# githubhjs/h264-jm-commentary

Hardware: AMD Instinct MI355X
Metric: ME+transform megapixels/sec @1080p FullSearch SR=32; bit-exact vs the in-repo JM restatement (oracle); device-resident (inputs in HBM, no H2D/D2H in the timed region) (higher is better)
Workload: dtype u8

## Files before the change

### h264-jm-commentary_amd/csrc/jmh_analyse.hip

```cpp
#include "jmh_common.h"
#include "jmh_launch.h"
#include "jmh_intra8.h"
#include "jmh_intra.h"
#include "jmh_i4.h"
#include "jmh_spiral.h"
#ifdef JMH_FLOW_TU
#include "jmh_final.h"
#endif

#define MVB_OFF 544
#define MVB_LEN 1104
#define MV_ABS_MAX (4 * 2 * SRMAX + 3)
#define MVB_ARG_MAX (4 * 2 * SRMAX + MV_ABS_MAX + 3)
static_assert(MVB_ARG_MAX == 518 && MVB_ARG_MAX <= MVB_OFF && MVB_OFF + MVB_ARG_MAX < MVB_LEN,
              "s.mvc holds every MV difference the full-pel and sub-pel searches can form at SRMAX");
#define PLS (WIN_DIM_MAX * WST + 32)
#define MAXNS 7

struct MeS {
    uint8_t org[256];
    Border bd;
    IntraNb<uint8_t> nb;
    int16_t all_mv[8][16][2];
    int motion_cost[8][4];
    unsigned red[NTA / 64][MAXNS];
    int pmv[MAXNS][2];
    uint16_t mvc[MVB_LEN];
    uint8_t planes[4 * PLS];
    union {
        int16_t h1[WIN_DIM_MAX * WST];
        uint2 sad8[NPK * NTA];
    } hs;
    gptr<unsigned long long> pst;
    int pn;
    alignas(8) IntraS<uint8_t> in;
};
union AnalyseS {
    MeS me;
    IntraS<uint8_t> in[4];
};

__device__ __forceinline__ void sstamp(MeS &s, int wave) {
    if (wave == 2 && __lane_id() == 0 && s.pst && s.pn < 44) s.pst[s.pn++] = wall_clock64();
}

struct NbMe {
    const MeS &s;
    int bt, b8, best8x8;
    __device__ bool operator()(int xN, int yN, int &ref, int &mx, int &my) const {
        if (yN > 15 || (xN > 15 && yN >= 0)) return false;
        if (xN < 0 || yN < 0) {
            int c = border_cell(xN, yN);
// ... 60 lines not shown
#pragma unroll
        for (int k = 0; k < NPK; k++) {
            const unsigned cost = psum<BT, BX, BY>(sp[k]) + cxv + cy[4 * k];
            const uint32_t o = ordk_of(ps, k);
            const bool in = max(rx, abs(ps.dy0 + k - sr)) <= range || o == 0;
            b = min(b, in ? (cost << 13) | o : 0xFFFFFFFFu);
        }
    }
    return b;
}

__device__ __forceinline__ int search_range(const DevParams &d, int bt) { return d.restrict_sr == 0 ? d.sr / min(2, bt) : d.sr; }

struct SDesc {
    int bt, bx4, by4, mc;
    int fbt, fbx4, fby4, fslot;
};

__device__ __forceinline__ uint32_t lds_u32_at(const uint8_t *p) { return lds_u32_any(p); }
typedef short s16x2 __attribute__((ext_vector_type(2)));
__device__ __forceinline__ s16x2 as_s2(uint32_t v) { return __builtin_bit_cast(s16x2, v); }
__device__ __forceinline__ uint32_t as_u32(s16x2 v) { return __builtin_bit_cast(uint32_t, v); }
__device__ __forceinline__ s16x2 abs2(s16x2 v) { return __builtin_elementwise_max(v, (s16x2)(0) - v); }
__device__ __forceinline__ s16x2 lo16(uint32_t w) { return as_s2(__builtin_amdgcn_perm(0u, w, 0x0c010c00u)); }
__device__ __forceinline__ s16x2 hi16(uint32_t w) { return as_s2(__builtin_amdgcn_perm(0u, w, 0x0c030c02u)); }
__device__ __forceinline__ s16x2 tap6_2(s16x2 a, s16x2 b, s16x2 c, s16x2 d, s16x2 e, s16x2 f) {
    return (a + f) + (s16x2)(20) * (c + d) - (s16x2)(5) * (b + e);
}
__device__ __forceinline__ s16x2 clip5(s16x2 v) {
    return __builtin_elementwise_min(__builtin_elementwise_max((v + (s16x2)(16)) >> (s16x2)(5), (s16x2)(0)), (s16x2)(255));
}
__device__ __forceinline__ uint32_t pack4(s16x2 lo, s16x2 hi) { return __builtin_amdgcn_perm(as_u32(hi), as_u32(lo), 0x06040200u); }

template <bool HALF>
__device__ __forceinline__ int subblock_satd(const MeS &s, int wbase, int obase, int ox, int oy, int had) {
    const int off = qoff((oy & 3) * 4 + (ox & 3));
    const int xa = (off >> 12) & 15, ya = (off >> 8) & 15, xb = (off >> 4) & 15, yb = off & 15;
    const int oA = ((xa & 1) + 2 * (ya & 1)) * PLS + (ya >> 1) * WST + (xa >> 1);
    const int oB = ((xb & 1) + 2 * (yb & 1)) * PLS + (yb >> 1) * WST + (xb >> 1);
    const uint8_t *r0 = s.planes + wbase + (oy >> 2) * WST + (ox >> 2);
    uint32_t O[4], P[4];
#pragma unroll
    for (int yy = 0; yy < 4; yy++) {
        const uint32_t A = lds_u32_at(r0 + yy * WST + oA);
        if constexpr (HALF) P[yy] = A;
        else {
            const uint32_t B = lds_u32_at(r0 + yy * WST + oB);
            P[yy] = (A | B) - (((A ^ B) >> 1) & 0x7F7F7F7Fu);
        }
        O[yy] = *reinterpret_cast<const uint32_t *>(s.org + obase + 16 * yy);
    }
    if (!had) {
        uint32_t sad = 0;
#pragma unroll
        for (int yy = 0; yy < 4; yy++) sad = __builtin_amdgcn_sad_u8(O[yy], P[yy], sad);
// ... 398 lines not shown
    }
    int minc = BIGCOST, c_mode = 0;
#pragma unroll
    for (int m = 0; m < 4; m++) {
        int c = 0;
#pragma unroll
        for (int q = 0; q < 8; q++) c += __builtin_amdgcn_readlane(sat, 8 * m + q);
        if (chroma_mode_ok(m, avL, avT, avTL) && c < minc) { minc = c; c_mode = m; }
    }
    if (lane == 0) scr->c_mode = c_mode;
}

template <class SC>
__device__ __forceinline__ void intra_slot(const DevParams &d, IntraS<uint8_t> &s, SC *scr, int16_t (*i4lev)[16], int k, int w, int mbx, int mby);

__device__ __forceinline__ void me_prologue(const DevParams &d, MeS &s, int mbx, int mby) {
    const int tid = threadIdx.x;
    if (tid < 256) s.in.org[tid] = s.org[tid] = d.orgY[(16 * mby + (tid >> 4)) * d.W + 16 * mbx + (tid & 15)];
    else if (tid >= 472 && tid < 478) s.in.part[(tid - 472) / 3][(tid - 472) % 3] = 0;
    else if (tid >= 480 && tid < 512) s.motion_cost[(tid - 480) >> 2][tid & 3] = 0;
    for (int i = tid; i < MVB_LEN; i += NTA) s.mvc[i] = (uint16_t)__umul24(d.lambda_motion, mvbits(i - MVB_OFF));
}

template <class SC>
__device__ __forceinline__ void me_mb(const DevParams &d, MeS &s, SC *scr, int16_t (*i4lev)[16], int mbx, int mby, bool pre = false) {
    const int tid = threadIdx.x;
    const int wave = __builtin_amdgcn_readfirstlane(tid >> 6);
    const int W = d.W, sr = d.sr, side = d.side;
    const int pix_x = 16 * mbx, pix_y = 16 * mby;
    const bool prof = prof_mb_here(d, mbx, mby);
    PSTAMP(0);
    if (tid == 0) { s.pst = prof ? d.prof + 20 : nullptr; s.pn = 0; }
    if (tid < 256) {
        if (!pre) s.in.org[tid] = s.org[tid] = d.orgY[(pix_y + (tid >> 4)) * W + pix_x + (tid & 15)];
        else if (tid >= 128 && tid < 199) load_intra_nb_batch(d, s.in.nb, tid - 128, mbx, mby);
    }
    else if (tid >= 384 && tid < 394) load_border(d, s.bd, tid - 384, mbx, mby, &s.in.bd);
    else if (!pre && tid >= 472 && tid < 478) s.in.part[(tid - 472) / 3][(tid - 472) % 3] = 0;
    else if (!pre && tid >= 480 && tid < 512) s.motion_cost[(tid - 480) >> 2][tid & 3] = 0;
    auto idle = [&](int k, int w) { intra_slot(d, s.in, scr, i4lev, k, w, mbx, mby); };
    if (!pre)
        for (int i = tid; i < MVB_LEN; i += NTA) s.mvc[i] = (uint16_t)__umul24(d.lambda_motion, mvbits(i - MVB_OFF));
    int pcx = 0, pcy = 0, scx = 0, scy = 0;
    uint8_t *G = s.planes;
    const int wdim = 2 * sr + 16 + 2 * WM;
    {
        __syncthreads();
        set_mvp(NbBorder{s.bd}, 0, 0, 16, 16, pcx, pcy);
        scx = iclip(-sr, sr, pcx / 4); scy = iclip(-sr, sr, pcy / 4);
        const int X0 = pix_x + scx - sr - WM, Y0 = pix_y + scy - sr - WM;
        constexpr int ND4 = WST / 4, NWT = (WIN_DIM_MAX * ND4 + NTA - 1) / NTA;
        uint32_t lo_[NWT], hi_[NWT];
        bool fast[NWT];
#pragma unroll
        for (int i = 0; i < NWT; i++) {
            const int task = tid + i * NTA;
            const int y = task / ND4, j = task - y * ND4, x0 = X0 + 4 * j;
            fast[i] = task < wdim * ND4 && 4 * j + 3 < wdim && x0 >= 0 && x0 + 3 < W;
            const int bx = iclip(0, W - 4, x0 & ~3);
            const gptr<const uint32_t> p = reinterpret_cast<gptr<const uint32_t>>(d.refY + iclip(0, d.H - 1, Y0 + y) * W + bx);
            lo_[i] = p[0];
            hi_[i] = ((x0 & 3) && bx + 4 < W) ? p[1] : 0u;
        }
#pragma unroll
        for (int i = 0; i < NWT; i++) {
            const int task = tid + i * NTA;
            if (task >= wdim * ND4) break;
            const int y = task / ND4, j = task - y * ND4, x0 = X0 + 4 * j;
            uint32_t v;
            if (fast[i]) v = __builtin_amdgcn_alignbyte(hi_[i], lo_[i], x0 & 3);
            else {
                const int bx = iclip(0, W - 4, x0 & ~3);
                v = 0;
#pragma unroll
                for (int q = 0; q < 4; q++) {
                    const int c = iclip(0, W - 1, x0 + q) - bx;
                    if (4 * j + q < wdim) v |= (((c < 4 ? lo_[i] : hi_[i]) >> (8 * (c & 3))) & 255u) << (8 * q);
                }
            }
            *reinterpret_cast<uint32_t *>(G + y * WST + 4 * j) = v;
        }
        if (tid < 32) G[wdim * WST + tid] = 0;
        if (!pre && tid >= 128 && tid < 199) load_intra_nb(d, s.in.nb, tid - 128, mbx, mby);
    }
    __syncthreads();
    PSTAMP(1);
    {
        PosState ps;
        const int nstrips = (side + NPK - 1) / NPK;
        const bool sact = tid < side * nstrips;
        ps.dx = sact ? tid % side : 0;
        ps.dy0 = sact ? (tid / side) * NPK : 0;
        ps.scx = scx; ps.scy = scy;
        PSTAMP(8);
#pragma unroll
        for (int k2 = 0; k2 < NPK2; k2++) ps.ordk2[k2] = d.ordtab[k2 * NTA + tid];
        {
            const int k0 = sr - scy - ps.dy0;
            const bool mine = sact && ps.dx == sr - scx;
#pragma unroll
            for (int k2 = 0; k2 < NPK2; k2++)
                if (mine && (k0 >> 1) == k2) ps.ordk2[k2] &= (k0 & 1) ? 0x0000FFFFu : 0xFFFF0000u;
        }
        PSTAMP(9);
        {
            const int lo = WM - 1, n = 2 * sr + 18;
            uint8_t *PB = s.planes + PLS, *PH = s.planes + 2 * PLS, *PJ = s.planes + 3 * PLS;
            constexpr int NG = WIN_DIM_MAX / 4, NR = NTA / NG;
            const int g = tid % NG, rb = tid / NG, c0 = 4 * g;
            const int run = (n + NR - 1) / NR, y0 = lo + rb * run, y1 = rb < NR ? min(lo + n, y0 + run) : y0;
            if (y0 < y1) {
                const uint32_t *gc = reinterpret_cast<const uint32_t *>(G + c0);
                constexpr int WS4 = WST / 4;
                uint32_t w0 = gc[(y0 - 2) * WS4], w1 = gc[(y0 - 1) * WS4], w2 = gc[y0 * WS4], w3 = gc[(y0 + 1) * WS4], w4 = gc[(y0 + 2) * WS4];
                for (int y = y0; y < y1; y++) {
                    const uint32_t w5 = gc[(y + 3) * WS4];
                    const uint32_t L = gc[y * WS4 - 1], R = gc[y * WS4 + 1];
                    int hv[4];
                    uint32_t ph = 0, pb = 0;
#pragma unroll
                    for (int i = 0; i < 4; i++) {
                        const int sh = 8 * i;
                        hv[i] = tap6((int)((w0 >> sh) & 255u), (int)((w1 >> sh) & 255u), (int)((w2 >> sh) & 255u), (int)((w3 >> sh) & 255u),
                                     (int)((w4 >> sh) & 255u), (int)((w5 >> sh) & 255u));
                        ph |= (uint32_t)clip255((hv[i] + 16) >> 5) << sh;
                    }
                    const uint64_t mr = ((uint64_t)R << 32) | w2;
                    int bx[9];
                    bx[0] = (int)((L >> 16) & 255u); bx[1] = (int)(L >> 24);
#pragma unroll
                    for (int k = 0; k < 7; k++) bx[2 + k] = (int)((mr >> (8 * k)) & 255u);
#pragma unroll
                    for (int i = 0; i < 4; i++)
                        pb |= (uint32_t)clip255((tap6(bx[i], bx[i + 1], bx[i + 2], bx[i + 3], bx[i + 4], bx[i + 5]) + 16) >> 5) << (8 * i);
#pragma unroll
                    for (int i = 0; i < 4; i++) {
                        const int cx = c0 + i;
                        s.hs.h1[y * WST + cx] = (int16_t)hv[i];
                        { PH[y * WST + cx] = (uint8_t)(ph >> (8 * i)); PB[y * WST + cx] = (uint8_t)(pb >> (8 * i)); }
                    }
                    w0 = w1; w1 = w2; w2 = w3; w3 = w4; w4 = w5;
                }
            }
            __syncthreads();
            PSTAMP(10);
            for (int y = y0; y < y1; y++) {
                const uint32_t *hr = reinterpret_cast<const uint32_t *>(s.hs.h1 + y * WST + c0);
                const uint32_t q0 = hr[-1], q1 = hr[0], q2 = hr[1], q3 = hr[2], q4 = hr[3];
                const int x[9] = {(int)(int16_t)q0, (int)q0 >> 16, (int)(int16_t)q1, (int)q1 >> 16, (int)(int16_t)q2,
                                  (int)q2 >> 16, (int)(int16_t)q3, (int)q3 >> 16, (int)(int16_t)q4};
                uint32_t jv = 0;
#pragma unroll
                for (int i = 0; i < 4; i++)
                    jv |= (uint32_t)clip255((tap6(x[i], x[i + 1], x[i + 2], x[i + 3], x[i + 4], x[i + 5]) + 512) >> 10) << (8 * i);
#pragma unroll
                for (int i = 0; i < 4; i++)
                    PJ[y * WST + c0 + i] = (uint8_t)(jv >> (8 * i));
            }
        }
        __syncthreads();
        PSTAMP(2);
        {
            int best8x8 = 0, cost8x8 = 0;
            p8x8_block<0>(d, s, ps, best8x8, cost8x8, idle, wave, tid);
            PSTAMP(3);
            p8x8_block<1>(d, s, ps, best8x8, cost8x8, idle, wave, tid);
            PSTAMP(4);
            p8x8_block<2>(d, s, ps, best8x8, cost8x8, idle, wave, tid);
            PSTAMP(5);
            p8x8_block<3>(d, s, ps, best8x8, cost8x8, idle, wave, tid);
            if constexpr (scr_global<SC>) {
                if (tid < 224) {
                    const int m = 1 + tid / 32, k = (tid & 31) >> 1, c = tid & 1;
                    scr->all_mv[m][k][c] = s.all_mv[m][k][c];
                } else if (tid < 252) {
                    const int m = 1 + (tid - 224) / 4, k = tid & 3;
                    scr->motion_cost[m][k] = s.motion_cost[m][k];
                }
            }
            if (tid == 256) {
                scr->best8x8 = best8x8; scr->cost8x8 = cost8x8;
            } else if (tid == 320) {
                NbBorder nbv{s.bd};
                int ra = -1, ax = 0, ay = 0, rb = -1, bx = 0, by = 0;
                const bool aa = nbv(-1, 0, ra, ax, ay), ab = nbv(0, -1, rb, bx, by);
                const bool zl = !aa || (ra == 0 && ax == 0 && ay == 0), za = !ab || (rb == 0 && bx == 0 && by == 0);
                scr->skipx = (za || zl) ? 0 : pcx;
                scr->skipy = (za || zl) ? 0 : pcy;
            }
            PSTAMP(6);
        }
    }
}

template <class pel, class SC>
__device__ __forceinline__ void intra_role(const DevParams &d, IntraS<pel> &s, SC *scr, int16_t (*i4lev)[16], int mbx, int mby, int tid, bool act,
                                           bool i4) {
    const int wave = tid >> 6, lane = tid & 63;
    const int pix_x = 16 * mbx, pix_y = 16 * mby, W = d.W;
    const MbAvail mav = intra_avail(d, mbx, mby);
    const bool avL = mav.L, avT = mav.T, avTL = mav.TL, avTR = mav.TR;
    const bool prof = act && prof_mb_here(d, mbx, mby);
    PSTAMP(12);
    if (act) {
        const gptr<const pel> orgY = spl<pel>(d.orgY);
        s.org[tid] = orgY[(pix_y + (tid >> 4)) * W + pix_x + (tid & 15)];
        s.org[tid + 128] = orgY[(pix_y + 8 + (tid >> 4)) * W + pix_x + (tid & 15)];
        load_orgc(d, s.nb, tid, mbx, mby);
        if (tid < 10) load_border(d, s.bd, tid, mbx, mby);
        else if (tid >= 16 && tid < 16 + 71) load_intra_nb(d, s.nb, tid - 16, mbx, mby);
    }
    const int q_bits = 15 + (d.qp + d.qpbd) / 6;
// ... 116 lines not shown
        const int mby = d.y_min + ((act ? q : t.pre[e]) - t.pre[e]), mbx = d.diag - 2 * mby;
        MbScratch *scr = d.scr + mby * d.mbw + mbx;
        intra_role(d, s.in[threadIdx.x >> 7], scr, scr->i4lev, mbx, mby, threadIdx.x & 127, act, true);
    } else {
        const int mi = xcd_block(b - nRg, tot);
        if (mi >= tot) return;
        intra8_mb<pel>(t, s.i8, mi);
    }
}

hipError_t jmh_launch_intra(const TickArgs &t, hipStream_t st) {
    const int tot = t.pre[t.npic];
    const int nblocks = xcd_grid((tot + 1) / 2) + (t.t8 ? xcd_grid(tot) : 0);
    if (t.bd > 8) hipLaunchKernelGGL(k_mb_intra<uint16_t>, dim3(nblocks), dim3(NT), 0, st, t);
    else hipLaunchKernelGGL(k_mb_intra<uint8_t>, dim3(nblocks), dim3(NT), 0, st, t);
    return hipGetLastError();
}

hipError_t jmh_launch_analyse(const TickArgs &t, hipStream_t st) {
    const int nPm = t.me_in_analyse ? t.pre[t.nP] : 0;
    const int nblocks = xcd_grid(nPm) + (t.pre[t.npic] + 3) / 4;
    if (nblocks == 0) return hipSuccess;
    hipLaunchKernelGGL(k_mb_analyse, dim3(nblocks), dim3(NTA), 0, st, t);
    return hipGetLastError();
}
#endif

#ifdef JMH_FLOW_TU
__device__ __forceinline__ int own_sgpr(int v) {
    asm("" : "+s"(v));
    return v;
}

__device__ __forceinline__ DevParams flow_params(const FlowArgs &f, const PicParams &q) {
    DevParams d;
    const int W = own_sgpr(f.W), H = own_sgpr(f.H), sr = own_sgpr(f.sr);
    d.W = W; d.H = H; d.Wc = W >> 1; d.Hc = H >> 1; d.mbw = own_sgpr(f.mbw); d.mbh = own_sgpr(f.mbh);
    d.sr = sr; d.side = 2 * sr + 1; d.npos = d.side * d.side;
    d.search_mode = own_sgpr(f.search_mode); d.use_hadamard = own_sgpr(f.use_hadamard); d.restrict_sr = own_sgpr(f.restrict_sr);
    d.isr = f.isr;
    d.t8 = 0;
    d.epzs_dual = 0; d.epzs_subpel = 0; d.epzs_spts = 0; d.epzs_mints = 0; d.epzs_maxts = 0;
    d.slice_mbs = f.slice_mbs;
    d.maxv = 255; d.qpbd = 0;
    const int ls = W * H, lc = ls >> 2;
    set_pic_pointers(d, q, ls, lc);
// ... 185 lines not shown
```

### h264-jm-commentary_amd/csrc/jmh_launch.h

```cpp
#pragma once
#include "jmh_device.h"

hipError_t jmh_launch_analyse(const TickArgs &t, hipStream_t st);
hipError_t jmh_launch_intra(const TickArgs &t, hipStream_t st);
hipError_t jmh_launch_flow(const FlowArgs &f, hipStream_t st);
hipError_t jmh_launch_intra8(const TickArgs &t, hipStream_t st);
hipError_t jmh_launch_me_full(const TickArgs &t, hipStream_t st);
hipError_t jmh_launch_epzs(const TickArgs &t, hipStream_t st);
hipError_t jmh_launch_final(const TickArgs &t, hipStream_t st);
hipError_t jmh_launch_rdo(const TickArgs &t, hipStream_t st, hipStream_t side, hipEvent_t fork, hipEvent_t join);
size_t jmh_rdo_scratch_bytes();
hipError_t jmh_launch_ingest(int format, const IngestArgs &a, hipStream_t st);
hipError_t jmh_launch_ingest_rgb(int format, const RgbArgs &a, hipStream_t st);
hipError_t jmh_launch_ingest_yuv(int format, const YuvArgs &a, hipStream_t st);
hipError_t jmh_launch_ingest_tensor(int dtype, const TensorArgs &a, hipStream_t st);
hipError_t jmh_launch_scale(const ScaleArgs &a, hipStream_t st);
hipError_t jmh_launch_pull_picture(int format, const OutArgs &a, hipStream_t st);
hipError_t jmh_launch_pull_tensor(int dtype, const OutArgs &a, hipStream_t st);

hipError_t jmh_launch_interp(const uint8_t *ref, int W, int H, uint8_t *qpel, int qstride, int qplane, hipStream_t st);
hipError_t jmh_launch_spiral_positions(int count, int32_t *out_xy, hipStream_t st);
template <class pel>
hipError_t jmh_launch_sad_table(const pel *org, const pel *ref, int W, int H, int sr, int n_mb, const int32_t *mb_xy, const int32_t *centres,
                                uint16_t *out, hipStream_t st);
template <class pel>
hipError_t jmh_launch_tq4x4(int n, const int16_t *resid, const pel *pred, int qpb, int qsel, int maxv, int16_t *levels, pel *recon,
                            int32_t *cc, int32_t *nz, hipStream_t st);
template <class pel>
hipError_t jmh_launch_tq8x8(int n, const int16_t *resid, const pel *pred, int qpb, int qsel, int maxv, int16_t *levels, pel *recon,
                            int32_t *cc, int32_t *nz, hipStream_t st);
template <class pel>
hipError_t jmh_launch_block_search(int n, const jmh_block_search *reqs, jmh_block_result *out, const pel *cur, const pel *ref, int W, int H,
                                   int had, int maxv, hipStream_t st);
```

### h264-jm-commentary_amd/csrc/jmhip_abi.hip

```cpp
#include <algorithm>
#include "jmh_ctx.h"
#include "jmh_spiral.h"

#define JMH_CODED_CAP_DEFAULT 192
#define JMW_MB_MAX_BYTES_ANY 16576

static int q_selector(const jmh_config &cfg, bool i_slice) {
    return cfg.jm_version >= 10 ? 2 + cfg.quant_offset[i_slice ? 0 : 1] : i_slice ? 1 : 0;
}

#define KT_STRIDE 32
static int ring_init(EvRing &r, int cap) {
    r.cap = cap; r.head = r.count = r.n = 0; r.sum = 0;
    r.a.assign(cap, nullptr); r.b.assign(cap, nullptr);
    for (int i = 0; i < cap; i++)
        if (hipEventCreate(&r.a[i]) != hipSuccess || hipEventCreate(&r.b[i]) != hipSuccess) return -1;
    return 0;
}
static void ring_free(EvRing &r) {
    for (int i = 0; i < r.cap; i++) {
        if (r.a[i]) (void)hipEventDestroy(r.a[i]);
        if (r.b[i]) (void)hipEventDestroy(r.b[i]);
    }
    r.cap = 0;
// ... 1381 lines not shown
    c->cabac_split = chunk_bins;
    return JMH_OK;
}
int jmh_cabac_get_split(const jmh_ctx *c) { return c ? c->cabac_split : JMH_E_INVALID_ARG; }
int jmh_cabac_split_stats(const jmh_ctx *c, jmh_cabac_split_info *out) {
    if (!c || !out) return JMH_E_INVALID_ARG;
    jmh_cabac_split_last(c->cabac, out);
    return JMH_OK;
}

int jmh_spiral_positions(jmh_ctx *c, int search_range, int32_t *out_xy) {
    if (!c || !out_xy || search_range < 1 || search_range > SRMAX) return JMH_E_INVALID_ARG;
    const int side = 2 * search_range + 1, count = side * side;
    HCHK(hipSetDevice(c->dev));
    DevTemps tmp;
    int32_t *d_out = nullptr;
    if (tmp.alloc(&d_out, (size_t)count * 2 * sizeof(int32_t)) != hipSuccess) return JMH_E_OOM;
    HCHK(jmh_launch_spiral_positions(count, d_out, c->st));
    HCHK(hipMemcpyAsync(out_xy, d_out, (size_t)count * 2 * sizeof(int32_t), hipMemcpyDeviceToHost, c->st));
    HCHK(hipStreamSynchronize(c->st));
    return JMH_OK;
}

int jmh_read_recon(jmh_ctx *c, uint8_t *y, uint8_t *u, uint8_t *v, int sy, int sc) { return read_pic(c, y, u, v, sy, sc, false, false); }
int jmh_read_recon_u16(jmh_ctx *c, uint16_t *y, uint16_t *u, uint16_t *v, int sy, int sc) { return read_pic(c, y, u, v, sy, sc, true, false); }
int jmh_read_deblocked(jmh_ctx *c, uint8_t *y, uint8_t *u, uint8_t *v, int sy, int sc) { return read_pic(c, y, u, v, sy, sc, false, true); }
int jmh_read_deblocked_u16(jmh_ctx *c, uint16_t *y, uint16_t *u, uint16_t *v, int sy, int sc) { return read_pic(c, y, u, v, sy, sc, true, true); }
int jmh_load_frame(jmh_ctx *c, int slot, const uint8_t *y, const uint8_t *u, const uint8_t *v, int sy, int sc) {
    return load_frame_any(c, slot, y, u, v, sy, sc, false);
}
int jmh_load_frame_u16(jmh_ctx *c, int slot, const uint16_t *y, const uint16_t *u, const uint16_t *v, int sy, int sc) {
    return load_frame_any(c, slot, y, u, v, sy, sc, true);
}

int jmh_encode_slot(jmh_ctx *c, int slot, const jmh_frame_params *fp) {
    if (!c || !fp || slot < 0 || slot >= c->nslots) return JMH_E_INVALID_ARG;
    int r = check_params(c, fp);
    if (r) return r;
    HCHK(hipSetDevice(c->dev));
    int e;
    if ((r = claim_entry(c, &e))) return r;
    c->ring[e].coded = 0;
    return push_picture(c, c->d_slots + (size_t)slot * c->fsize, e, fp, 0);
}

int jmh_sync(jmh_ctx *c) {
// ... 161 lines not shown
```

### h264-jm-commentary_amd/jmhip.py

```python
import ctypes
import os

import numpy as np

HERE = os.path.dirname(os.path.abspath(__file__))
LIB_PATH = os.environ.get("JMH_LIB_PATH") or os.path.join(HERE, "csrc", "libjmhip.so")
HOST_LIB_PATH = os.path.join(HERE, "host", "build", "libjmhost.so")

JMH_OK = 0
JMH_E_INVALID_ARG, JMH_E_HIP, JMH_E_OOM, JMH_E_UNSUPPORTED_CFG, JMH_E_STATE, JMH_E_NO_DEVICE = -1, -2, -3, -4, -5, -6
JMH_P_SLICE, JMH_I_SLICE = 0, 2
JMH_ABI_VERSION = 14
JMH_FLAG_KERNEL_TIMING = 1
STATUS = {0: "ok", -1: "invalid argument", -2: "HIP runtime error", -3: "out of memory",
          -4: "unsupported configuration", -5: "invalid call order", -6: "no HIP device"}
QP2QUANT = [1, 1, 1, 1, 2, 2, 2, 2, 3, 3, 3, 4, 4, 4, 5, 6, 6, 7, 8, 9, 10, 11, 13, 14, 16, 18,
            20, 23, 25, 29, 32, 36, 40, 45, 51, 57, 64, 72, 81, 91]


def lambda_rdo_off(qp):
    return QP2QUANT[max(0, qp - 12)]


def lambda_rdo_on(qp, bit_depth=8):
# ... 291 lines not shown
}
EXPORTED_OUTPUT = tuple(_SIGS_OUTPUT)

JMH_SCALE_OFF, JMH_SCALE_BILINEAR, JMH_SCALE_BICUBIC, JMH_SCALE_LANCZOS3 = 0, 1, 2, 3
JMH_SCALE_CHROMA_LEFT = 1
JMH_SCALE_TAPS_MAX, JMH_SCALE_SRC_MAX = 24, 8192


class JmhScale(ctypes.Structure):
    _fields_ = [("filter", ctypes.c_int32), ("flags", ctypes.c_int32), ("out_width", ctypes.c_int32), ("out_height", ctypes.c_int32)]


_SIGS_SCALE = {
    "jmh_input_scale": (_I, [_P, _P]),
    "jmh_scale_taps": (_I, [_I, _I, _I, _I, _P, _P, _P]),
    "jmh_scale_info": (_I, [_P, _P, _P]),
}
EXPORTED_SCALE = tuple(_SIGS_SCALE)

_SIGS_SPIRAL = {
    "jmh_spiral_positions": (_I, [_P, _I, _P]),
}
EXPORTED_SPIRAL = tuple(_SIGS_SPIRAL)


def scale_taps(n_src, n_dst, filter, chroma_left=False):
    lib = load()
    nt = ctypes.c_int(0)
    st = lib.jmh_scale_taps(n_src, n_dst, filter, int(bool(chroma_left)), None, None, ctypes.byref(nt))
    _check(st, "jmh_scale_taps")
    first = np.empty(n_dst, np.int32)
    taps = np.empty((n_dst, nt.value), np.int16)
    _check(lib.jmh_scale_taps(n_src, n_dst, filter, int(bool(chroma_left)), _ptr(first), _ptr(taps), ctypes.byref(nt)), "jmh_scale_taps")
    return first, taps


def rgb_coefficients(format, bit_depth):
    out = (ctypes.c_int32 * 12)()
    _check(load().jmh_rgb_coefficients(format, bit_depth, out), "jmh_rgb_coefficients")
    return [int(v) for v in out]


def _tensor_dtype(a, dtype=None):
    if dtype is not None:
        if a.dtype.itemsize != TENSOR_ELEM_BYTES[dtype]:
            raise ValueError(f"elements of {a.dtype.itemsize} bytes do not hold dtype {dtype}")
# ... 869 lines not shown
        res = np.ascontiguousarray(res, MB_RESULT_DTYPE)
        if res.size != self.mbw * self.mbh:
            raise JmhError(f"cabac_results: {res.size} results for {self.mbw * self.mbh} macroblocks")
        return self._cabac(lambda *a: self.lib.jmh_cabac_write_results(self.ctx, _ptr(res), *a), "jmh_cabac_write_results", descs, cap,
                           with_where)

    def cabac_split(self, chunk_bins):
        _check(self.lib.jmh_cabac_set_split(self.ctx, int(chunk_bins)), "jmh_cabac_set_split")

    def cabac_split_info(self):
        info = JmhCabacSplitInfo()
        _check(self.lib.jmh_cabac_split_stats(self.ctx, ctypes.byref(info)), "jmh_cabac_split_stats")
        return dict(chunk_bins=info.chunk_bins, chunks=info.chunks, longest_slice_chunks=info.longest_slice_chunks,
                    scratch_bytes=info.scratch_bytes, setting=self.lib.jmh_cabac_get_split(self.ctx))

    def spiral_positions(self, search_range):
        fn = self.lib.jmh_spiral_positions
        fn.restype, fn.argtypes = _SIGS_SPIRAL["jmh_spiral_positions"]
        side = 2 * search_range + 1
        out = np.empty((side * side, 2), np.int32)
        _check(fn(self.ctx, search_range, _ptr(out)), "jmh_spiral_positions")
        return out

    def sad_table(self, mb_xy, centres):
        mb_xy = np.ascontiguousarray(mb_xy, np.int32)
        centres = np.ascontiguousarray(centres, np.int32)
        n = mb_xy.shape[0]
        side = 2 * self.cfg.search_range + 1
        out = np.empty((n, 16, side * side), np.uint16)
        _check(self.lib.jmh_ffs_sad_table(self.ctx, n, _ptr(mb_xy), _ptr(centres), _ptr(out)),
               "jmh_ffs_sad_table")
        return out

    def tq4x4(self, resid, pred, qp, intra):
        resid = np.ascontiguousarray(resid, np.int16)
        pred = np.ascontiguousarray(pred, np.uint8)
        n = resid.shape[0]
        lev = np.empty((n, 16), np.int16)
        rec = np.empty((n, 16), np.uint8)
        cc = np.empty(n, np.int32)
        nz = np.empty(n, np.int32)
        _check(self.lib.jmh_tq4x4_batch(self.ctx, n, _ptr(resid), _ptr(pred), qp, intra, _ptr(lev),
                                        _ptr(rec), _ptr(cc), _ptr(nz)), "jmh_tq4x4_batch")
        return lev, rec, cc, nz

    def tq8x8(self, resid, pred, qp, intra):
# ... 144 lines not shown
```

### include/jmhip.h

```cpp
#ifndef JMHIP_H
#define JMHIP_H

#include <stdint.h>

#ifdef __cplusplus
extern "C" {
#endif

#define JMH_ABI_VERSION 14
#define JMH_LAMBDA_MAX 1023
#define JMH_QOFFSET_MAX 2047

#define JMH_OK                 0
#define JMH_E_INVALID_ARG     (-1)
#define JMH_E_HIP             (-2)
#define JMH_E_OOM             (-3)
#define JMH_E_UNSUPPORTED_CFG (-4)
#define JMH_E_STATE           (-5)
#define JMH_E_NO_DEVICE       (-6)

#define JMH_P_SLICE 0
#define JMH_I_SLICE 2

#define JMH_PSKIP  0
// ... 169 lines not shown
                          int stride_y, int stride_c, const jmh_frame_params *fp);
int  jmh_frame_push_u16(jmh_ctx *ctx, const uint16_t *y, const uint16_t *u, const uint16_t *v,
                        int stride_y, int stride_c, const jmh_frame_params *fp);
int  jmh_read_recon_u16(jmh_ctx *ctx, uint16_t *y, uint16_t *u, uint16_t *v, int stride_y, int stride_c);
int  jmh_read_deblocked_u16(jmh_ctx *ctx, uint16_t *y, uint16_t *u, uint16_t *v, int stride_y, int stride_c);
int  jmh_load_frame_u16(jmh_ctx *ctx, int slot, const uint16_t *y, const uint16_t *u, const uint16_t *v,
                        int stride_y, int stride_c);

int  jmh_read_qpel(jmh_ctx *ctx, uint8_t *out);

#ifdef __cplusplus
}
#endif
#include "jmhip_cavlc.h"
#include "jmhip_cabac.h"
#include "jmhip_coded.h"
#include "jmhip_cabac_split.h"
#include "jmhip_input.h"
#include "jmhip_nal.h"
#include "jmhip_rgb.h"
#include "jmhip_yuv.h"
#include "jmhip_tensor.h"
#include "jmhip_spiral.h"
#include "jmhip_scale.h"
#include "jmhip_output.h"
#endif
```

Baseline: 1538.

## Vectorise half-pel plane interpolation with packed 16-bit math and LDS addressing

Moves the search-window load and the half-pel plane (b, h, j) generation into shared helpers. The per-byte scalar 6-tap filter is replaced with packed s16x2 arithmetic using byte-permute, and LDS accesses go through explicit 32-bit LDS addresses with 64-bit writes of the h1 intermediate. The skip-MV computation moves earlier so it runs during the window load rather than after the search. It also adds a standalone window-planes kernel and ABI entry point for testing, which brings extra code and new alignment requirements on the shared-memory struct.

```diff
diff --git a/h264-jm-commentary_amd/csrc/jmh_analyse.hip b/h264-jm-commentary_amd/csrc/jmh_analyse.hip
--- a/h264-jm-commentary_amd/csrc/jmh_analyse.hip
+++ b/h264-jm-commentary_amd/csrc/jmh_analyse.hip
@@ -4,6 +4,7 @@
 #include "jmh_intra.h"
 #include "jmh_i4.h"
 #include "jmh_spiral.h"
+#include "jmh_planes.h"
 #ifdef JMH_FLOW_TU
 #include "jmh_final.h"
 #endif
@@ -26,8 +27,8 @@
     unsigned red[NTA / 64][MAXNS];
     int pmv[MAXNS][2];
     uint16_t mvc[MVB_LEN];
-    uint8_t planes[4 * PLS];
-    union {
+    alignas(4) uint8_t planes[4 * PLS];
+    alignas(8) union {
         int16_t h1[WIN_DIM_MAX * WST];
         uint2 sad8[NPK * NTA];
     } hs;
@@ -134,15 +135,6 @@
 __device__ __forceinline__ s16x2 as_s2(uint32_t v) { return __builtin_bit_cast(s16x2, v); }
 __device__ __forceinline__ uint32_t as_u32(s16x2 v) { return __builtin_bit_cast(uint32_t, v); }
 __device__ __forceinline__ s16x2 abs2(s16x2 v) { return __builtin_elementwise_max(v, (s16x2)(0) - v); }
-__device__ __forceinline__ s16x2 lo16(uint32_t w) { return as_s2(__builtin_amdgcn_perm(0u, w, 0x0c010c00u)); }
-__device__ __forceinline__ s16x2 hi16(uint32_t w) { return as_s2(__builtin_amdgcn_perm(0u, w, 0x0c030c02u)); }
-__device__ __forceinline__ s16x2 tap6_2(s16x2 a, s16x2 b, s16x2 c, s16x2 d, s16x2 e, s16x2 f) {
-    return (a + f) + (s16x2)(20) * (c + d) - (s16x2)(5) * (b + e);
-}
-__device__ __forceinline__ s16x2 clip5(s16x2 v) {
-    return __builtin_elementwise_min(__builtin_elementwise_max((v + (s16x2)(16)) >> (s16x2)(5), (s16x2)(0)), (s16x2)(255));
-}
-__device__ __forceinline__ uint32_t pack4(s16x2 lo, s16x2 hi) { return __builtin_amdgcn_perm(as_u32(hi), as_u32(lo), 0x06040200u); }
 
 template <bool HALF>
 __device__ __forceinline__ int subblock_satd(const MeS &s, int wbase, int obase, int ox, int oy, int had) {
@@ -587,6 +579,91 @@
     for (int i = tid; i < MVB_LEN; i += NTA) s.mvc[i] = (uint16_t)__umul24(d.lambda_motion, mvbits(i - MVB_OFF));
 }
 
+__device__ __forceinline__ void window_load(gptr<const uint8_t> refY, int W, int H, int X0, int Y0, int wdim, uint8_t *G, int tid) {
+    constexpr int ND4 = WST / 4, NWT = (WIN_DIM_MAX * ND4 + NTA - 1) / NTA;
+    uint32_t lo_[NWT], hi_[NWT];
+    bool fast[NWT];
+#pragma unroll
+    for (int i = 0; i < NWT; i++) {
+        const int task = tid + i * NTA;
+        const int y = task / ND4, j = task - y * ND4, x0 = X0 + 4 * j;
+        fast[i] = task < wdim * ND4 && 4 * j + 3 < wdim && x0 >= 0 && x0 + 3 < W;
+        const int bx = iclip(0, W - 4, x0 & ~3);
+        const gptr<const uint32_t> p = reinterpret_cast<gptr<const uint32_t>>(refY + iclip(0, H - 1, Y0 + y) * W + bx);
+        lo_[i] = p[0];
+        hi_[i] = ((x0 & 3) && bx + 4 < W) ? p[1] : 0u;
+    }
+#pragma unroll
+    for (int i = 0; i < NWT; i++) {
+        const int task = tid + i * NTA;
+        if (task >= wdim * ND4) break;
+        const int y = task / ND4, j = task - y * ND4, x0 = X0 + 4 * j;
+        uint32_t v;
+        if (fast[i]) v = __builtin_amdgcn_alignbyte(hi_[i], lo_[i], x0 & 3);
+        else {
+            const int bx = iclip(0, W - 4, x0 & ~3);
+            v = 0;
+#pragma unroll
+            for (int q = 0; q < 4; q++) {
+                const int c = iclip(0, W - 1, x0 + q) - bx;
+                if (4 * j + q < wdim) v |= (((c < 4 ? lo_[i] : hi_[i]) >> (8 * (c & 3))) & 255u) << (8 * q);
+            }
+        }
+        *reinterpret_cast<uint32_t *>(G + y * WST + 4 * j) = v;
+    }
+    if (tid < 32) G[wdim * WST + tid] = 0;
+}
+
+struct PlaneMap {
+    uint32_t c0, y0, y1;
+};
+__device__ __forceinline__ PlaneMap plane_map(int sr, int tid) {
+    const uint32_t lo = WM - 1, n = 2 * sr + 18;
+    constexpr uint32_t NG = WIN_DIM_MAX / 4, NR = NTA / NG;
+    const uint32_t g = (uint32_t)tid % NG, rb = (uint32_t)tid / NG;
+    const uint32_t run = (n + NR - 1) / NR, y0 = lo + __umul24(rb, run);
+    return {4 * g, y0, rb < NR ? min(lo + n, y0 + run) : y0};
+}
+
+typedef __attribute__((address_space(3))) uint32_t lds_u32;
+typedef uint32_t u32x2 __attribute__((ext_vector_type(2)));
+typedef __attribute__((address_space(3))) u32x2 lds_u2;
+typedef __attribute__((address_space(3))) const u32x2 lds_cu2;
+__device__ __forceinline__ uint32_t lds_addr(const void *p) { return (uint32_t)(uintptr_t)(lds_cu8 *)p; }
+__device__ __forceinline__ uint32_t lds_rd32(uint32_t a) { return *(lds_cu32 *)(uintptr_t)a; }
+__device__ __forceinline__ u32x2 lds_rd64(uint32_t a) { return *(lds_cu2 *)(uintptr_t)a; }
+__device__ __forceinline__ void lds_wr32(uint32_t a, uint32_t v) { *(lds_u32 *)(uintptr_t)a = v; }
+__device__ __forceinline__ void lds_wr64(uint32_t a, u32x2 v) { *(lds_u2 *)(uintptr_t)a = v; }
+
+__device__ __forceinline__ void planes_h1hb(MeS &s, const PlaneMap pm) {
+    if (pm.y0 >= pm.y1) return;
+    const uint32_t ro = __umul24(pm.y0, WST) + pm.c0;
+    uint32_t g = lds_addr(s.planes) + ro, h1 = lds_addr(s.hs.h1) + 2 * ro;
+    uint32_t w0 = lds_rd32(g - 2 * WST), w1 = lds_rd32(g - WST), w2 = lds_rd32(g), w3 = lds_rd32(g + WST), w4 = lds_rd32(g + 2 * WST);
+    for (uint32_t y = pm.y0; y < pm.y1; y++, g += WST, h1 += 2 * WST) {
+        const uint32_t w5 = lds_rd32(g + 3 * WST);
+        const uint32_t L = lds_rd32(g - 4), R = lds_rd32(g + 4);
+        jmp_u64 hv;
+        uint32_t hh, bb;
+        jmp_row_h1hb(w0, w1, w2, w3, w4, w5, L, R, &hv, &hh, &bb);
+        lds_wr64(h1, u32x2{hv.lo, hv.hi});
+        lds_wr32(g + 2 * PLS, hh);
+        lds_wr32(g + PLS, bb);
+        w0 = w1; w1 = w2; w2 = w3; w3 = w4; w4 = w5;
+    }
+}
+
+__device__ __forceinline__ void planes_j(MeS &s, const PlaneMap pm) {
+    if (pm.y0 >= pm.y1) return;
+    const uint32_t ro = __umul24(pm.y0, WST) + pm.c0;
+    uint32_t j = lds_addr(s.planes) + 3 * PLS + ro, h1 = lds_addr(s.hs.h1) + 2 * ro;
+    for (uint32_t y = pm.y0; y < pm.y1; y++, j += WST, h1 += 2 * WST) {
+        const uint32_t q0 = lds_rd32(h1 - 4);
+        const u32x2 a = lds_rd64(h1), b = lds_rd64(h1 + 8);
+        lds_wr32(j, jmp_row_j(q0, a.x, a.y, b.x, b.y));
+    }
+}
+
 template <class SC>
 __device__ __forceinline__ void me_mb(const DevParams &d, MeS &s, SC *scr, int16_t (*i4lev)[16], int mbx, int mby, bool pre = false) {
     const int tid = threadIdx.x;
@@ -612,40 +689,16 @@
     {
         __syncthreads();
         set_mvp(NbBorder{s.bd}, 0, 0, 16, 16, pcx, pcy);
-        scx = iclip(-sr, sr, pcx / 4); scy = iclip(-sr, sr, pcy / 4);
-        const int X0 = pix_x + scx - sr - WM, Y0 = pix_y + scy - sr - WM;
-        constexpr int ND4 = WST / 4, NWT = (WIN_DIM_MAX * ND4 + NTA - 1) / NTA;
-        uint32_t lo_[NWT], hi_[NWT];
-        bool fast[NWT];
-#pragma unroll
-        for (int i = 0; i < NWT; i++) {
-            const int task = tid + i * NTA;
-            const int y = task / ND4, j = task - y * ND4, x0 = X0 + 4 * j;
-            fast[i] = task < wdim * ND4 && 4 * j + 3 < wdim && x0 >= 0 && x0 + 3 < W;
-            const int bx = iclip(0, W - 4, x0 & ~3);
-            const gptr<const uint32_t> p = reinterpret_cast<gptr<const uint32_t>>(d.refY + iclip(0, d.H - 1, Y0 + y) * W + bx);
-            lo_[i] = p[0];
-            hi_[i] = ((x0 & 3) && bx + 4 < W) ? p[1] : 0u;
-        }
-#pragma unroll
-        for (int i = 0; i < NWT; i++) {
-            const int task = tid + i * NTA;
-            if (task >= wdim * ND4) break;
-            const int y = task / ND4, j = task - y * ND4, x0 = X0 + 4 * j;
-            uint32_t v;
-            if (fast[i]) v = __builtin_amdgcn_alignbyte(hi_[i], lo_[i], x0 & 3);
-            else {
-                const int bx = iclip(0, W - 4, x0 & ~3);
-                v = 0;
-#pragma unroll
-                for (int q = 0; q < 4; q++) {
-                    const int c = iclip(0, W - 1, x0 + q) - bx;
-                    if (4 * j + q < wdim) v |= (((c < 4 ? lo_[i] : hi_[i]) >> (8 * (c & 3))) & 255u) << (8 * q);
-                }
-            }
-            *reinterpret_cast<uint32_t *>(G + y * WST + 4 * j) = v;
-        }
-        if (tid < 32) G[wdim * WST + tid] = 0;
+        scx = __builtin_amdgcn_readfirstlane(iclip(-sr, sr, pcx / 4)); scy = iclip(-sr, sr, pcy / 4);
+        if (tid == 320) {
+            NbBorder nbv{s.bd};
+            int ra = -1, ax = 0, ay = 0, rb = -1, bx = 0, by = 0;
+            const bool aa = nbv(-1, 0, ra, ax, ay), ab = nbv(0, -1, rb, bx, by);
+            const bool zl = !aa || (ra == 0 && ax == 0 && ay == 0), za = !ab || (rb == 0 && bx == 0 && by == 0);
+            scr->skipx = (za || zl) ? 0 : pcx;
+            scr->skipy = (za || zl) ? 0 : pcy;
+        }
+        window_load(d.refY, W, d.H, pix_x + scx - sr - WM, pix_y + scy - sr - WM, wdim, G, tid);
         if (!pre && tid >= 128 && tid < 199) load_intra_nb(d, s.in.nb, tid - 128, mbx, mby);
     }
     __syncthreads();
@@ -669,59 +722,11 @@
         }
         PSTAMP(9);
         {
-            const int lo = WM - 1, n = 2 * sr + 18;
-            uint8_t *PB = s.planes + PLS, *PH = s.planes + 2 * PLS, *PJ = s.planes + 3 * PLS;
-            constexpr int NG = WIN_DIM_MAX / 4, NR = NTA / NG;
-            const int g = tid % NG, rb = tid / NG, c0 = 4 * g;
-            const int run = (n + NR - 1) / NR, y0 = lo + rb * run, y1 = rb < NR ? min(lo + n, y0 + run) : y0;
-            if (y0 < y1) {
-                const uint32_t *gc = reinterpret_cast<const uint32_t *>(G + c0);
-                constexpr int WS4 = WST / 4;
-                uint32_t w0 = gc[(y0 - 2) * WS4], w1 = gc[(y0 - 1) * WS4], w2 = gc[y0 * WS4], w3 = gc[(y0 + 1) * WS4], w4 = gc[(y0 + 2) * WS4];
-                for (int y = y0; y < y1; y++) {
-                    const uint32_t w5 = gc[(y + 3) * WS4];
-                    const uint32_t L = gc[y * WS4 - 1], R = gc[y * WS4 + 1];
-                    int hv[4];
-                    uint32_t ph = 0, pb = 0;
-#pragma unroll
-                    for (int i = 0; i < 4; i++) {
-                        const int sh = 8 * i;
-                        hv[i] = tap6((int)((w0 >> sh) & 255u), (int)((w1 >> sh) & 255u), (int)((w2 >> sh) & 255u), (int)((w3 >> sh) & 255u),
-                                     (int)((w4 >> sh) & 255u), (int)((w5 >> sh) & 255u));
-                        ph |= (uint32_t)clip255((hv[i] + 16) >> 5) << sh;
-                    }
-                    const uint64_t mr = ((uint64_t)R << 32) | w2;
-                    int bx[9];
-                    bx[0] = (int)((L >> 16) & 255u); bx[1] = (int)(L >> 24);
-#pragma unroll
-                    for (int k = 0; k < 7; k++) bx[2 + k] = (int)((mr >> (8 * k)) & 255u);
-#pragma unroll
-                    for (int i = 0; i < 4; i++)
-                        pb |= (uint32_t)clip255((tap6(bx[i], bx[i + 1], bx[i + 2], bx[i + 3], bx[i + 4], bx[i + 5]) + 16) >> 5) << (8 * i);
-#pragma unroll
-                    for (int i = 0; i < 4; i++) {
-                        const int cx = c0 + i;
-                        s.hs.h1[y * WST + cx] = (int16_t)hv[i];
-                        { PH[y * WST + cx] = (uint8_t)(ph >> (8 * i)); PB[y * WST + cx] = (uint8_t)(pb >> (8 * i)); }
-                    }
-                    w0 = w1; w1 = w2; w2 = w3; w3 = w4; w4 = w5;
-                }
-            }
+            const PlaneMap pm = plane_map(sr, tid);
+            planes_h1hb(s, pm);
             __syncthreads();
             PSTAMP(10);
-            for (int y = y0; y < y1; y++) {
-                const uint32_t *hr = reinterpret_cast<const uint32_t *>(s.hs.h1 + y * WST + c0);
-                const uint32_t q0 = hr[-1], q1 = hr[0], q2 = hr[1], q3 = hr[2], q4 = hr[3];
-                const int x[9] = {(int)(int16_t)q0, (int)q0 >> 16, (int)(int16_t)q1, (int)q1 >> 16, (int)(int16_t)q2,
-                                  (int)q2 >> 16, (int)(int16_t)q3, (int)q3 >> 16, (int)(int16_t)q4};
-                uint32_t jv = 0;
-#pragma unroll
-                for (int i = 0; i < 4; i++)
-                    jv |= (uint32_t)clip255((tap6(x[i], x[i + 1], x[i + 2], x[i + 3], x[i + 4], x[i + 5]) + 512) >> 10) << (8 * i);
-#pragma unroll
-                for (int i = 0; i < 4; i++)
-                    PJ[y * WST + c0 + i] = (uint8_t)(jv >> (8 * i));
-            }
+            planes_j(s, pm);
         }
         __syncthreads();
         PSTAMP(2);
@@ -743,16 +748,7 @@
                     scr->motion_cost[m][k] = s.motion_cost[m][k];
                 }
             }
-            if (tid == 256) {
-                scr->best8x8 = best8x8; scr->cost8x8 = cost8x8;
-            } else if (tid == 320) {
-                NbBorder nbv{s.bd};
-                int ra = -1, ax = 0, ay = 0, rb = -1, bx = 0, by = 0;
-                const bool aa = nbv(-1, 0, ra, ax, ay), ab = nbv(0, -1, rb, bx, by);
-                const bool zl = !aa || (ra == 0 && ax == 0 && ay == 0), za = !ab || (rb == 0 && bx == 0 && by == 0);
-                scr->skipx = (za || zl) ? 0 : pcx;
-                scr->skipy = (za || zl) ? 0 : pcy;
-            }
+            if (tid == 256) { scr->best8x8 = best8x8; scr->cost8x8 = cost8x8; }
             PSTAMP(6);
         }
     }
@@ -915,6 +911,28 @@
     const int nblocks = xcd_grid(nPm) + (t.pre[t.npic] + 3) / 4;
     if (nblocks == 0) return hipSuccess;
     hipLaunchKernelGGL(k_mb_analyse, dim3(nblocks), dim3(NTA), 0, st, t);
+    return hipGetLastError();
+}
+
+__global__ __launch_bounds__(NTA) void k_window_planes(const uint8_t *ref, int W, int H, int X0, int Y0, int sr, uint8_t *out) {
+    __shared__ MeS s;
+    const int tid = threadIdx.x, wdim = 2 * sr + 16 + 2 * WM;
+    for (int i = tid; i < PLS; i += NTA) reinterpret_cast<uint32_t *>(s.planes)[i] = 0;
+    __syncthreads();
+    window_load(to_global(ref), W, H, X0, Y0, wdim, s.planes, tid);
+    __syncthreads();
+    const PlaneMap pm = plane_map(sr, tid);
+    planes_h1hb(s, pm);
+    __syncthreads();
+    planes_j(s, pm);
+    __syncthreads();
+    for (int i = tid; i < 4 * wdim * wdim; i += NTA) {
+        const int p = i / (wdim * wdim), r = i - p * wdim * wdim, y = r / wdim, x = r - y * wdim;
+        out[i] = s.planes[p * PLS + y * WST + x];
+    }
+}
+hipError_t jmh_launch_window_planes(const uint8_t *ref, int W, int H, int X0, int Y0, int sr, uint8_t *out, hipStream_t st) {
+    hipLaunchKernelGGL(k_window_planes, dim3(1), dim3(NTA), 0, st, ref, W, H, X0, Y0, sr, out);
     return hipGetLastError();
 }
 #endif
diff --git a/h264-jm-commentary_amd/csrc/jmh_launch.h b/h264-jm-commentary_amd/csrc/jmh_launch.h
--- a/h264-jm-commentary_amd/csrc/jmh_launch.h
+++ b/h264-jm-commentary_amd/csrc/jmh_launch.h
@@ -20,6 +20,7 @@
 
 hipError_t jmh_launch_interp(const uint8_t *ref, int W, int H, uint8_t *qpel, int qstride, int qplane, hipStream_t st);
 hipError_t jmh_launch_spiral_positions(int count, int32_t *out_xy, hipStream_t st);
+hipError_t jmh_launch_window_planes(const uint8_t *ref, int W, int H, int X0, int Y0, int sr, uint8_t *out, hipStream_t st);
 template <class pel>
 hipError_t jmh_launch_sad_table(const pel *org, const pel *ref, int W, int H, int sr, int n_mb, const int32_t *mb_xy, const int32_t *centres,
                                 uint16_t *out, hipStream_t st);
diff --git a/h264-jm-commentary_amd/csrc/jmh_planes.h b/h264-jm-commentary_amd/csrc/jmh_planes.h
--- /dev/null
+++ b/h264-jm-commentary_amd/csrc/jmh_planes.h
@@ -0,0 +1,79 @@
+#ifndef JMH_PLANES_H
+#define JMH_PLANES_H
+#include <stdint.h>
+
+#if defined(__HIPCC__)
+#define JMP_FN __host__ __device__ static __forceinline__
+#else
+#define JMP_FN static inline
+#endif
+
+typedef short jmp_s2 __attribute__((vector_size(4)));
+typedef struct { uint32_t lo, hi; } jmp_u64;
+
+#if defined(__HIP_DEVICE_COMPILE__)
+#define JMP_PAIR(hi, lo, i, k) jmp_as_s2(__builtin_amdgcn_perm((hi), (lo), 0x0c000c00u | (uint32_t)(i) | ((uint32_t)(k) << 16)))
+#else
+#define JMP_PAIR(hi, lo, i, k) jmp_pair_host((hi), (lo), (i), (k))
+#endif
+JMP_FN jmp_s2 jmp_as_s2(uint32_t v) { jmp_s2 r; __builtin_memcpy(&r, &v, 4); return r; }
+JMP_FN uint32_t jmp_as_u32(jmp_s2 v) { uint32_t r; __builtin_memcpy(&r, &v, 4); return r; }
+JMP_FN jmp_s2 jmp_pair_host(uint32_t hi, uint32_t lo, int i, int k) {
+    const uint64_t w = ((uint64_t)hi << 32) | lo;
+    return jmp_as_s2((uint32_t)((w >> (8 * i)) & 255u) | (uint32_t)((w >> (8 * k)) & 255u) << 16);
+}
+JMP_FN jmp_s2 jmp_splat(int v) { jmp_s2 r = {(short)v, (short)v}; return r; }
+JMP_FN jmp_s2 jmp_clamp255(jmp_s2 v) {
+#if defined(__HIP_DEVICE_COMPILE__)
+    return __builtin_elementwise_min(__builtin_elementwise_max(v, jmp_splat(0)), jmp_splat(255));
+#else
+    const jmp_s2 z = jmp_splat(0), m = jmp_splat(255);
+    v = v & ~(v < z);
+    return (v & (v < m)) | (m & ~(v < m));
+#endif
+}
+JMP_FN uint32_t jmp_pack4(jmp_s2 a, jmp_s2 b) {
+#if defined(__HIP_DEVICE_COMPILE__)
+    return __builtin_amdgcn_perm(jmp_as_u32(b), jmp_as_u32(a), 0x06040200u);
+#else
+    const uint32_t x = jmp_as_u32(a), y = jmp_as_u32(b);
+    return (x & 255u) | ((x >> 16) & 255u) << 8 | (y & 255u) << 16 | ((y >> 16) & 255u) << 24;
+#endif
+}
+
+JMP_FN jmp_s2 jmp_tap6_2(jmp_s2 a, jmp_s2 b, jmp_s2 c, jmp_s2 d, jmp_s2 e, jmp_s2 f) {
+    return (c + d) * jmp_splat(20) + (a + f) + (b + e) * jmp_splat(-5);
+}
+JMP_FN jmp_s2 jmp_clip5(jmp_s2 v) { return jmp_clamp255((v + jmp_splat(16)) >> jmp_splat(5)); }
+
+JMP_FN void jmp_row_h1hb(uint32_t w0, uint32_t w1, uint32_t w2, uint32_t w3, uint32_t w4, uint32_t w5, uint32_t L, uint32_t R,
+                         jmp_u64 *h1, uint32_t *h, uint32_t *b) {
+    const jmp_s2 v01 = jmp_tap6_2(JMP_PAIR(0u, w0, 0, 1), JMP_PAIR(0u, w1, 0, 1), JMP_PAIR(0u, w2, 0, 1), JMP_PAIR(0u, w3, 0, 1),
+                                  JMP_PAIR(0u, w4, 0, 1), JMP_PAIR(0u, w5, 0, 1));
+    const jmp_s2 v23 = jmp_tap6_2(JMP_PAIR(0u, w0, 2, 3), JMP_PAIR(0u, w1, 2, 3), JMP_PAIR(0u, w2, 2, 3), JMP_PAIR(0u, w3, 2, 3),
+                                  JMP_PAIR(0u, w4, 2, 3), JMP_PAIR(0u, w5, 2, 3));
+    h1->lo = jmp_as_u32(v01);
+    h1->hi = jmp_as_u32(v23);
+    *h = jmp_pack4(jmp_clip5(v01), jmp_clip5(v23));
+    const jmp_s2 p0 = JMP_PAIR(w2, L, 2, 3), p1 = JMP_PAIR(w2, L, 3, 4), p2 = JMP_PAIR(0u, w2, 0, 1), p3 = JMP_PAIR(0u, w2, 1, 2),
+                 p4 = JMP_PAIR(0u, w2, 2, 3), p5 = JMP_PAIR(R, w2, 3, 4), p6 = JMP_PAIR(0u, R, 0, 1), p7 = JMP_PAIR(0u, R, 1, 2);
+    *b = jmp_pack4(jmp_clip5(jmp_tap6_2(p0, p1, p2, p3, p4, p5)), jmp_clip5(jmp_tap6_2(p2, p3, p4, p5, p6, p7)));
+}
+
+JMP_FN int jmp_tap6(int a, int b, int c, int d, int e, int f) { return a - 5 * b + 20 * c + 20 * d - 5 * e + f; }
+JMP_FN int jmp_clip255(int v) { return v < 0 ? 0 : (v > 255 ? 255 : v); }
+JMP_FN uint32_t jmp_row_j(uint32_t q0, uint32_t q1, uint32_t q2, uint32_t q3, uint32_t q4) {
+    const int x[9] = {(int)(int16_t)q0, (int)q0 >> 16, (int)(int16_t)q1, (int)q1 >> 16, (int)(int16_t)q2,
+                      (int)q2 >> 16,    (int)(int16_t)q3, (int)q3 >> 16, (int)(int16_t)q4};
+    uint32_t jv = 0;
+    for (int i = 0; i < 4; i++) {
+        int v = (jmp_tap6(x[i], x[i + 1], x[i + 2], x[i + 3], x[i + 4], x[i + 5]) + 512) >> 10;
+#if defined(__HIP_DEVICE_COMPILE__)
+        asm("" : "+v"(v));
+#endif
+        jv |= (uint32_t)jmp_clip255(v) << (8 * i);
+    }
+    return jv;
+}
+
+#endif
diff --git a/h264-jm-commentary_amd/csrc/jmhip_abi.hip b/h264-jm-commentary_amd/csrc/jmhip_abi.hip
--- a/h264-jm-commentary_amd/csrc/jmhip_abi.hip
+++ b/h264-jm-commentary_amd/csrc/jmhip_abi.hip
@@ -1427,6 +1427,25 @@
     return JMH_OK;
 }
 
+int jmh_window_planes(jmh_ctx *c, const uint8_t *ref_y, int W, int H, int x0, int y0, int search_range, uint8_t *out) {
+    if (!c || !ref_y || !out) return JMH_E_INVALID_ARG;
+    if (W <= 0 || H <= 0 || (W & 15) || (H & 15) || W > 16384 || H > 16384) return JMH_E_INVALID_ARG;
+    if (search_range < 1 || search_range > SRMAX) return JMH_E_INVALID_ARG;
+    constexpr int WM = 4;
+    if (x0 < -(2 * search_range + WM) || x0 > W - 16 - WM || y0 < -(2 * search_range + WM) || y0 > H - 16 - WM) return JMH_E_INVALID_ARG;
+    const int wdim = 2 * search_range + 16 + 2 * WM;
+    const size_t npic = (size_t)W * H, nout = (size_t)4 * wdim * wdim;
+    HCHK(hipSetDevice(c->dev));
+    DevTemps tmp;
+    uint8_t *d_ref = nullptr, *d_out = nullptr;
+    if (tmp.alloc(&d_ref, npic) != hipSuccess || tmp.alloc(&d_out, nout) != hipSuccess) return JMH_E_OOM;
+    HCHK(hipMemcpyAsync(d_ref, ref_y, npic, hipMemcpyHostToDevice, c->st));
+    HCHK(jmh_launch_window_planes(d_ref, W, H, x0, y0, search_range, d_out, c->st));
+    HCHK(hipMemcpyAsync(out, d_out, nout, hipMemcpyDeviceToHost, c->st));
+    HCHK(hipStreamSynchronize(c->st));
+    return JMH_OK;
+}
+
 int jmh_read_recon(jmh_ctx *c, uint8_t *y, uint8_t *u, uint8_t *v, int sy, int sc) { return read_pic(c, y, u, v, sy, sc, false, false); }
 int jmh_read_recon_u16(jmh_ctx *c, uint16_t *y, uint16_t *u, uint16_t *v, int sy, int sc) { return read_pic(c, y, u, v, sy, sc, true, false); }
 int jmh_read_deblocked(jmh_ctx *c, uint8_t *y, uint8_t *u, uint8_t *v, int sy, int sc) { return read_pic(c, y, u, v, sy, sc, false, true); }
diff --git a/h264-jm-commentary_amd/jmhip.py b/h264-jm-commentary_amd/jmhip.py
--- a/h264-jm-commentary_amd/jmhip.py
+++ b/h264-jm-commentary_amd/jmhip.py
@@ -337,6 +337,11 @@
     "jmh_spiral_positions": (_I, [_P, _I, _P]),
 }
 EXPORTED_SPIRAL = tuple(_SIGS_SPIRAL)
+
+_SIGS_PLANES = {
+    "jmh_window_planes": (_I, [_P, _P, _I, _I, _I, _I, _I, _P]),
+}
+EXPORTED_PLANES = tuple(_SIGS_PLANES)
 
 
 def scale_taps(n_src, n_dst, filter, chroma_left=False):
@@ -1252,6 +1257,16 @@
         _check(fn(self.ctx, search_range, _ptr(out)), "jmh_spiral_positions")
         return out
 
+    def window_planes(self, ref_y, x0, y0, search_range):
+        fn = self.lib.jmh_window_planes
+        fn.restype, fn.argtypes = _SIGS_PLANES["jmh_window_planes"]
+        ref_y = np.ascontiguousarray(ref_y, np.uint8)
+        h, w = ref_y.shape
+        wdim = 2 * search_range + 24
+        out = np.empty((4, wdim, wdim), np.uint8)
+        _check(fn(self.ctx, _ptr(ref_y), w, h, int(x0), int(y0), int(search_range), _ptr(out)), "jmh_window_planes")
+        return out
+
     def sad_table(self, mb_xy, centres):
         mb_xy = np.ascontiguousarray(mb_xy, np.int32)
         centres = np.ascontiguousarray(centres, np.int32)
diff --git a/include/jmhip.h b/include/jmhip.h
--- a/include/jmhip.h
+++ b/include/jmhip.h
@@ -215,6 +215,7 @@
 #include "jmhip_yuv.h"
 #include "jmhip_tensor.h"
 #include "jmhip_spiral.h"
+#include "jmhip_planes.h"
 #include "jmhip_scale.h"
 #include "jmhip_output.h"
 #endif
diff --git a/include/jmhip_planes.h b/include/jmhip_planes.h
--- /dev/null
+++ b/include/jmhip_planes.h
@@ -0,0 +1,15 @@
+#ifndef JMHIP_PLANES_H
+#define JMHIP_PLANES_H
+
+#include <stdint.h>
+
+#ifdef __cplusplus
+extern "C" {
+#endif
+
+int  jmh_window_planes(jmh_ctx *c, const uint8_t *ref_y, int W, int H, int x0, int y0, int search_range, uint8_t *out);
+
+#ifdef __cplusplus
+}
+#endif
+#endif
```

Result: no change. 1545 (median of 6 runs) (+0.4%).
